# Princic-1837592/julia-raytracer

Hardware: AMD Instinct MI355X
Metric: Mrays/s + wall-clock render time, cornellbox 1280×720×256spp (higher is better)
Workload: dtype f32; 1 GPU; cornellbox path 1280x720x256spp; scene=cornellbox, sampler=path, width=1280, height=720, spp=256, bounces=8, batch=256, traversal=near, traversal_requested=auto, bvh=middle, parallelism=1 tile groups x 1 sample ranges + RCCL reduce

## Files before the change

### julia-raytracer_amd/csrc/jt_bsdf.h

```cpp
#pragma once

#include "jt_device.h"

namespace jtd {

enum { M_MATTE = 0, M_GLOSSY, M_REFLECTIVE, M_TRANSPARENT, M_REFRACTIVE, M_SUBSURFACE, M_VOLUMETRIC, M_GLTFPBR };

struct MatPoint {
    int type;
    v3 emission, color;
    float opacity, roughness, metallic, ior;
    v3 density, scattering;
    float scanisotropy, trdepth;
};

__device__ __forceinline__ v3 up_normal(v3 normal, v3 outgoing) { return dot(normal, outgoing) <= 0 ? -normal : normal; }

__device__ __forceinline__ float fresnel_dielectric(float eta, v3 normal, v3 outgoing) {
    float cosw = __builtin_fabsf(dot(normal, outgoing));
    float sin2 = 1 - cosw * cosw;
    float eta2 = eta * eta;
    float cos2t = 1 - sin2 / eta2;
    if (cos2t < 0) return 1;
    float t0 = __builtin_sqrtf(cos2t);
// ... 24 lines not shown
    float sin2 = jl_clamp(1 - cos2, 0.0f, 1.0f);
    return V3(fresnel_conductor1(eta.x, 0.0f, cosw, cos2, sin2), fresnel_conductor1(eta.y, 0.0f, cosw, cos2, sin2),
              fresnel_conductor1(eta.z, 0.0f, cosw, cos2, sin2));
}
__device__ __forceinline__ v3 reflectivity_to_eta(v3 r) {
    float a = __builtin_sqrtf(jl_clamp(r.x, 0.0f, 0.99f));
    float b = __builtin_sqrtf(jl_clamp(r.y, 0.0f, 0.99f));
    float c = __builtin_sqrtf(jl_clamp(r.z, 0.0f, 0.99f));
    return V3((1 + a) / (1 - a), (1 + b) / (1 - b), (1 + c) / (1 - c));
}
__device__ __forceinline__ m3 basis_fromz(v3 v) {
    v3 z = normalize(v);
    float sign = __builtin_copysignf(1.0f, z.z);
    float a = -1.0f / (sign + z.z);
    float b = z.x * z.y * a;
    return m3{V3(1.0f + sign * z.x * z.x * a, sign * b, -sign * z.x), V3(b, sign + z.y * z.y * a, -z.y), z};
}
__device__ __forceinline__ v3 sample_hemisphere_cos(v3 normal, v2 ruv) {
    float z = __builtin_sqrtf(ruv.y);
    float r = __builtin_sqrtf(1 - z * z);
    float phi = 2 * pif * ruv.x;
    float s, c;
    jl_sincos(phi, &s, &c);
    v3 local = V3(r * c, r * s, z);
    return normalize(mul(basis_fromz(normal), local));
}
__device__ __forceinline__ v3 sample_sphere(v2 ruv) {
    float z = 2 * ruv.y - 1;
    float r = __builtin_sqrtf(jl_clamp(1 - z * z, 0.0f, 1.0f));
    float phi = 2 * pif * ruv.x;
    float s, c;
    jl_sincos(phi, &s, &c);
    return normalize(V3(r * c, r * s, z));
}
__device__ __forceinline__ float microfacet_distribution(float roughness, v3 normal, v3 halfway) {
    float cosine = dot(normal, halfway);
    if (cosine <= 0) return 0;
    float r2 = roughness * roughness;
    float c2 = cosine * cosine;
    return r2 / (pif * (c2 * r2 + 1 - c2) * (c2 * r2 + 1 - c2));
}
__device__ __forceinline__ float microfacet_shadowing1(float roughness, v3 normal, v3 halfway, v3 direction) {
    float cosine = dot(normal, direction);
    float cosineh = dot(halfway, direction);
    if (cosine * cosineh <= 0) return 0;
    float r2 = roughness * roughness;
    float c2 = cosine * cosine;
    return 2 * __builtin_fabsf(cosine) / (__builtin_fabsf(cosine) + __builtin_sqrtf(c2 - r2 * c2 + r2));
}
__device__ __forceinline__ float microfacet_shadowing(float roughness, v3 normal, v3 halfway, v3 outgoing,
                                                      v3 incoming) {
    return microfacet_shadowing1(roughness, normal, halfway, outgoing) *
           microfacet_shadowing1(roughness, normal, halfway, incoming);
}
__device__ __forceinline__ v3 sample_microfacet(float roughness, v3 normal, v2 rn) {
    float phi = 2 * pif * rn.x;
    float theta = jl_atan(roughness * __builtin_sqrtf(rn.y / (1 - rn.y)));
    float sp, cp, st, ct;
    jl_sincos(phi, &sp, &cp);
    jl_sincos(theta, &st, &ct);
    v3 local = V3(cp * st, sp * st, ct);
    return normalize(mul(basis_fromz(normal), local));
}
__device__ __forceinline__ float sample_microfacet_pdf(float roughness, v3 normal, v3 halfway) {
    float cosine = dot(normal, halfway);
    if (cosine < 0) return 0;
// ... 243 lines not shown
}
template <int F>
__device__ __forceinline__ void eval_bsdfcos_pdf(const MatPoint& m, v3 n, v3 o, v3 i, v3& f, float& pdf) {
    f = V3(0, 0, 0);
    pdf = 0;
    if (m.roughness == 0) return;
    switch (m.type) {
        case M_MATTE:
            f = eval_matte(m.color, n, o, i);
            pdf = sample_matte_pdf(n, o, i);
            return;
        case M_GLOSSY:
            f = eval_glossy(m.color, m.ior, m.roughness, n, o, i);
            pdf = sample_glossy_pdf(m.ior, m.roughness, n, o, i);
            return;
        case M_REFLECTIVE:
            f = eval_reflective(m.color, m.roughness, n, o, i);
            pdf = sample_reflective_pdf(m.roughness, n, o, i);
            return;
        case M_TRANSPARENT:
            f = eval_transparent(m.color, m.ior, m.roughness, n, o, i);
            pdf = sample_transparent_pdf(m.ior, m.roughness, n, o, i);
            return;
        case M_REFRACTIVE:
        case M_SUBSURFACE:
            if (F & FT_VOL) {
                f = eval_refractive(m.ior, m.roughness, n, o, i);
                pdf = sample_refractive_pdf(m.ior, m.roughness, n, o, i);
            }
            return;
        default: return;
    }
}
template <int F>
__device__ __forceinline__ v3 eval_delta(const MatPoint& m, v3 n, v3 o, v3 i) {
    if (m.roughness != 0) return V3(0, 0, 0);
    switch (m.type) {
        case M_REFLECTIVE: return eval_reflective_delta(m.color, n, o, i);
        case M_TRANSPARENT: return eval_transparent_delta(m.color, m.ior, n, o, i);
        case M_REFRACTIVE: return (F & FT_VOL) ? eval_refractive_delta(m.ior, n, o, i) : V3(0, 0, 0);
        case M_VOLUMETRIC:
            return ((F & FT_VOL) && !(dot(n, i) * dot(n, o) >= 0)) ? V3(1, 1, 1) : V3(0, 0, 0);
        default: return V3(0, 0, 0);
    }
}
template <int F>
__device__ __forceinline__ v3 sample_delta(const MatPoint& m, v3 n, v3 o, float rnl) {
    if (m.roughness != 0) return V3(0, 0, 0);
    switch (m.type) {
        case M_REFLECTIVE: return reflect(o, up_normal(n, o));
        case M_TRANSPARENT: return sample_transparent_delta(m.ior, n, o, rnl);
        case M_REFRACTIVE: return (F & FT_VOL) ? sample_refractive_delta(m.ior, n, o, rnl) : V3(0, 0, 0);
        case M_VOLUMETRIC: return -o;
        default: return V3(0, 0, 0);
    }
}
template <int F>
__device__ __forceinline__ float sample_delta_pdf(const MatPoint& m, v3 n, v3 o, v3 i) {
    if (m.roughness != 0) return 0;
    switch (m.type) {
        case M_REFLECTIVE: return dot(n, i) * dot(n, o) <= 0 ? 0.0f : 1.0f;
        case M_TRANSPARENT: return sample_transparent_delta_pdf(m.ior, n, o, i);
        case M_REFRACTIVE: return (F & FT_VOL) ? sample_refractive_delta_pdf(m.ior, n, o, i) : 0.0f;
        case M_VOLUMETRIC: return dot(n, i) * dot(n, o) >= 0 ? 0.0f : 1.0f;
        default: return 0;
    }
// ... 63 lines not shown
```

### julia-raytracer_amd/csrc/jt_integrator.h

```cpp
#pragma once

#include <hip/hip_runtime.h>

#include "jt_bsdf.h"
#include "jt_device.h"
#include "jt_launch.h"
#include "jt_scene_eval.h"
#include "jt_traverse.h"

#ifndef JT_FUSED_BSDF
#define JT_FUSED_BSDF 1
#endif

namespace jtk {
using namespace jtd;

template <int F>
__device__ __forceinline__ v3 sample_lights(const DScene& S, v3 position, float rl, float rel, v2 ruv) {
    const int light_id = sample_uniform(S.nlights, rl);
    const DLight l = S.lights[light_id - 1];
    const float* cdf = S.cdf + l.cdf_offset;
    if (l.instance >= 0) {
        const int element = l.nguide ? sample_discrete_guided(cdf, l.ncdf, rel, S.guide_t + l.guide_offset,
                                                              S.guide_a + l.guide_offset, l.nguide, l.guide_scale)
// ... 256 lines not shown
        if (light_hit<F>(S, P, st, query_hit(T))) return true;
    } while (st.phase == PH_LIGHT);
    return false;
}

struct Aov {
    float* acc;
    float w_;
    int first_;
    int lk_;
    template <int F>
    __device__ __forceinline__ float w() const {
        if (!lane_lds(F)) return w_;
        if (ft_none(F)) return jl_rcp_weight((float)(((reinterpret_cast<const int*>(acc)[11 * BLOCK] - first_) >> lk_) + 1));
        return acc[12 * BLOCK];
    }
};
template <int F>
__device__ __forceinline__ void aov_update(const Aov& a, v3 ta, v3 tn) {
    const float aw = a.w<F>();
    const float omw = 1 - aw;
    float* p = a.acc;
    p[4 * BLOCK] = p[4 * BLOCK] * omw + ta.x * aw;
    p[5 * BLOCK] = p[5 * BLOCK] * omw + ta.y * aw;
    p[6 * BLOCK] = p[6 * BLOCK] * omw + ta.z * aw;
    p[7 * BLOCK] = p[7 * BLOCK] * omw + tn.x * aw;
    p[8 * BLOCK] = p[8 * BLOCK] * omw + tn.y * aw;
    p[9 * BLOCK] = p[9 * BLOCK] * omw + tn.z * aw;
}
struct NoAov {};
template <int F>
__device__ __forceinline__ void aov_update(const NoAov&, v3, v3) {}

template <int F, class AovT>
__device__ __forceinline__ bool path_hit(const DScene& S, const DParams& P, Path& st, Hit isec, const AovT& aov,
                                         unsigned& shades) {
    if (!isec.hit) {
        if (st.bounce() > 0 || !P.envhidden)
            st.set_radiance<F>(st.radiance<F>() + st.weight<F>() * eval_environment<F>(S, st.d));
        return true;
    }
    bool in_volume = false;
    if ((F & FT_VOL) && st.flag(F_VOLUME)) {
        float rl = rand1f(st.rng), rd = rand1f(st.rng);
        float distance = sample_transmittance(st.vol.density, isec.t, rl, rd);
        v3 tr = eval_transmittance(st.vol.density, distance);
        float tp = sample_transmittance_pdf(st.vol.density, distance, isec.t);
        st.set_weight<F>((st.weight<F>() * tr) / tp);
        in_volume = distance < isec.t;
        isec.t = distance;
    }
    if (!in_volume) {
        v3 outgoing = -st.d;
        Shading sh;
        eval_shading<F>(S, isec.inst, isec.elem, V2(isec.u, isec.v), outgoing, sh);
        shades++;
        if (P.nocaustics) {
            st.set_max_roughness<F>(jl_max(sh.mat.roughness, st.max_roughness<F>()));
            sh.mat.roughness = st.max_roughness<F>();
        }
        if ((F & FT_OPAC) && sh.mat.opacity < 1 && rand1f(st.rng) >= sh.mat.opacity) {
            if (st.opbounce() > 128) return true;
            st.ctl += 1u << CTL_OPB;
            st.o = sh.position + st.d * 0.01f;
            return next_bounce_retry(P, st);
        }
        if (st.bounce() == 0) {
            st.set_flag(F_HIT);
            aov_update<F>(aov, sh.mat.color, sh.normal);
        }
        st.set_radiance<F>(st.radiance<F>() + st.weight<F>() * (dot(sh.normal, outgoing) >= 0 ? sh.mat.emission : V3(0, 0, 0)));
        v3 incoming;
        const bool delta = is_delta(sh.mat);
        if (!delta) {
            if (rand1f(st.rng) < 0.5f) {
                float rnl = rand1f(st.rng);
                v2 rn = rand2f(st.rng);
                incoming = sample_bsdfcos<F>(sh.mat, sh.normal, outgoing, rnl, rn);
            } else {
                float rl = rand1f(st.rng), rel = rand1f(st.rng);
                v2 ruv = rand2f(st.rng);
                incoming = sample_lights<F>(S, sh.position, rl, rel, ruv);
            }
            if (is_zero(incoming)) return true;
#if JT_FUSED_BSDF
            v3 fb;
            float pbv;
            eval_bsdfcos_pdf<F>(sh.mat, sh.normal, outgoing, incoming, fb, pbv);
            st.set_weight<F>(st.weight<F>() * fb);
            st.set_pb<F>(pbv);
#else
            st.set_weight<F>(st.weight<F>() * eval_bsdfcos<F>(sh.mat, sh.normal, outgoing, incoming));
            st.set_pb<F>(sample_bsdfcos_pdf<F>(sh.mat, sh.normal, outgoing, incoming));
#endif
        } else {
            float rnl = rand1f(st.rng);
            incoming = sample_delta<F>(sh.mat, sh.normal, outgoing, rnl);
            v3 f = eval_delta<F>(sh.mat, sh.normal, outgoing, incoming);
            float pd = sample_delta_pdf<F>(sh.mat, sh.normal, outgoing, incoming);
            st.set_weight<F>((st.weight<F>() * f) / pd);
        }
        const int mtype = sh.mat.type;
        if ((F & FT_VOL) && (mtype == M_REFRACTIVE || mtype == M_VOLUMETRIC || mtype == M_SUBSURFACE) &&
            dot(sh.normal, outgoing) * dot(sh.normal, incoming) < 0) {
            if (!st.flag(F_VOLUME)) {
                st.set_flag(F_VOLUME);
                st.vol.density = sh.mat.density;
                st.vol.scattering = sh.mat.scattering;
                st.vol.scanisotropy = sh.mat.scanisotropy;
            } else {
                st.clear_flag(F_VOLUME);
            }
        }
        st.o = sh.position;
        st.d = incoming;
        return delta ? after_weight<F>(P, st) : begin_light_pdf<F>(S, P, st);
    }
    v3 outgoing = -st.d;
    v3 position = st.o + st.d * isec.t;
    v3 incoming;
    if (rand1f(st.rng) < 0.5f) {
        (void)rand1f(st.rng);
        v2 rn = rand2f(st.rng);
        incoming = sample_scattering(st.vol, outgoing, rn);
    } else {
        float rl = rand1f(st.rng), rel = rand1f(st.rng);
        v2 ruv = rand2f(st.rng);
        incoming = sample_lights<F>(S, position, rl, rel, ruv);
    }
    if (is_zero(incoming)) return true;
    st.set_weight<F>(st.weight<F>() * eval_scattering(st.vol, outgoing, incoming));
    st.set_pb<F>(sample_scattering_pdf(st.vol, outgoing, incoming));
    st.o = position;
    st.d = incoming;
    return begin_light_pdf<F>(S, P, st);
}

template <int F, class AovT>
__device__ __forceinline__ bool naive_hit(const DScene& S, const DParams& P, Path& st, Hit isec, const AovT& aov,
                                          unsigned& shades) {
    if (!isec.hit) {
        if (st.bounce() > 0 || !P.envhidden)
            st.set_radiance<F>(st.radiance<F>() + st.weight<F>() * eval_environment<F>(S, st.d));
        return true;
    }
    v3 outgoing = -st.d;
    Shading sh;
    eval_shading<F>(S, isec.inst, isec.elem, V2(isec.u, isec.v), outgoing, sh);
    shades++;
    if ((F & FT_OPAC) && sh.mat.opacity < 1 && rand1f(st.rng) >= sh.mat.opacity) {
        if (st.opbounce() > 128) return true;
        st.ctl += 1u << CTL_OPB;
        st.o = sh.position + st.d * 0.01f;
        return next_bounce_retry(P, st);
    }
    if (st.bounce() == 0) {
        st.set_flag(F_HIT);
        aov_update<F>(aov, sh.mat.color, sh.normal);
    }
    st.set_radiance<F>(st.radiance<F>() + st.weight<F>() * (dot(sh.normal, outgoing) >= 0 ? sh.mat.emission : V3(0, 0, 0)));
    v3 incoming, f;
    float p;
    if (sh.mat.roughness != 0) {
        float rnl = rand1f(st.rng);
        v2 rn = rand2f(st.rng);
        incoming = sample_bsdfcos<F>(sh.mat, sh.normal, outgoing, rnl, rn);
        if (is_zero(incoming)) return true;
#if JT_FUSED_BSDF
        eval_bsdfcos_pdf<F>(sh.mat, sh.normal, outgoing, incoming, f, p);
#else
        f = eval_bsdfcos<F>(sh.mat, sh.normal, outgoing, incoming);
        p = sample_bsdfcos_pdf<F>(sh.mat, sh.normal, outgoing, incoming);
#endif
    } else {
        float rnl = rand1f(st.rng);
        incoming = sample_delta<F>(sh.mat, sh.normal, outgoing, rnl);
        if (is_zero(incoming)) return true;
        f = eval_delta<F>(sh.mat, sh.normal, outgoing, incoming);
        p = sample_delta_pdf<F>(sh.mat, sh.normal, outgoing, incoming);
    }
    st.set_weight<F>((st.weight<F>() * f) / p);
    st.o = sh.position;
    st.d = incoming;
    return after_weight<F>(P, st);
}

__device__ __forceinline__ void eval_camera(const DCamera& cam, v2 image_uv, v2 lens_uv, v3& ro, v3& rd) {
    const fr3 frame = frame_from(cam.frame);
    const v2 film = V2(cam.film_x, cam.film_y);
    if (!cam.orthographic) {
        v3 q = V3(film.x * (0.5f - image_uv.x), film.y * (image_uv.y - 0.5f), cam.lens);
        v3 dc = -normalize(q);
        v3 e = V3(lens_uv.x * cam.aperture / 2, lens_uv.y * cam.aperture / 2, 0);
        v3 p = (dc * cam.focus) / __builtin_fabsf(dc.z);
        v3 d = normalize(p - e);
        ro = transform_point(frame, e);
        rd = transform_direction(frame, d);
    } else {
        float scale = 1 / cam.lens;
        v3 q = V3(film.x * (0.5f - image_uv.x) * scale, film.y * (image_uv.y - 0.5f) * scale, cam.lens);
        v3 e = V3(-q.x, -q.y, 0) + V3(lens_uv.x * cam.aperture / 2, lens_uv.y * cam.aperture / 2, 0);
        v3 p = V3(-q.x, -q.y, -cam.focus);
// ... 34 lines not shown
```

### julia-raytracer_amd/csrc/jt_kernels.h

```cpp
#pragma once

#include <hip/hip_runtime.h>

#include <algorithm>

#include "jt_integrator.h"
#include "jt_launch.h"

namespace jtk {
using namespace jtd;

#ifndef JT_STAMPS
#define JT_STAMPS 0
#endif
#ifndef JT_NODE_REPEAT_NONE
#define JT_NODE_REPEAT_NONE 4
#endif
#ifndef JT_NODE_REPEAT
#define JT_NODE_REPEAT 3
#endif
#ifndef JT_FIRST_POP_NONE
#define JT_FIRST_POP_NONE 1
#endif
#ifndef JT_FIRST_POP
// ... 114 lines not shown
template <int F>
__device__ __forceinline__ unsigned item_of(int ut, int l, int i, int j) {
    return item_coords<F>() ? item_encode(i, j) : (unsigned)(ut * 64 + l);
}
template <int F>
__device__ __forceinline__ int item_pixel_index(unsigned item, const DParams& P, int tiles_x) {
    return item_coords<F>() ? item_j(item) * P.width + item_i(item) : item_pixel(item, P, tiles_x);
}
template <int F>
__device__ __forceinline__ int item_slot(unsigned item, const DParams& P) {
    if constexpr (item_coords<F>()) return item_slot(item, (P.width + 7) >> 3, P.tile_offset, P.tile_stride_rcp);
    else {
        const float inv = __uint_as_float(__builtin_amdgcn_readfirstlane(__float_as_uint(1.0f / (float)P.tile_stride)));
        return launch_tile((int)(item >> 6), P.tile_offset, inv) * 64 + (int)(item & 63u);
    }
}
__device__ __forceinline__ float stream_weight(const DParams& P, int s) {
    return jl_rcp_weight((float)(((s - P.first) >> P.lk) + 1));
}

#if JT_STAMPS
#define JT_STAMP(x) x
#else
#define JT_STAMP(x)
#endif

template <int SAMPLER, int RING, bool OVF, int COUNT, int F, bool NCACHE, bool WIDE, bool ADAPT = false>
__device__ __forceinline__ void trace_body_items(const DScene& S0, const DParams& P0, int s_begin, int s_end,
                                                 const DAccum& A, int* stack) {
    const DScene& S = S0;
    const DParams& P = P0;
    static_assert(lane_lds(F), "the per-lane item body keeps the lane's sample index in LDS");
    constexpr int PB = push_bit(node_baked<OVF, NCACHE, WIDE, F>());
    const int lane = threadIdx.x & 63;
    const int oslot = (int)blockIdx.x * BLOCK + (int)threadIdx.x;
    if constexpr ((F & (FT_TEX | FT_ENV)) != 0) {
        for (int k = threadIdx.x; k < 512; k += BLOCK) tex_lut[k] = k < 256 ? S.srgb_lut[k] : S.byte_lut[k - 256];
        __syncthreads();
    }
    Counters cnt{0, 0, 0, 0};
    constexpr bool WC = !ft_none(F);
    unsigned w_paths = 0, w_rays = 0, w_lq = 0;
    __shared__ unsigned wave_cnt[WC ? 1 : (BLOCK / 64) * 4];
    unsigned* const wcnt = wave_cnt + (WC ? 0 : (threadIdx.x >> 6) * 4);
    if (!WC && lane < 3) wcnt[lane] = 0u;
    auto lds_count = [&](int k, bool c) {
        if (c) __hip_atomic_fetch_add(wcnt + k, 1u, __ATOMIC_RELAXED, __HIP_MEMORY_SCOPE_WORKGROUP);
    };
    __shared__ float acc_lds[acc_slots(F) * BLOCK];
    float* acc = acc_lds + threadIdx.x;
    int* const acc_i = reinterpret_cast<int*>(acc);
#if JT_STAMPS
    unsigned long long t_trav = 0, t_shade = 0, n_trav = 0, n_shade = 0, lanes_p = 0, lanes_n = 0, steps_p = 0, steps_n = 0;
    unsigned long long t_hit = 0, t_fin = 0, t_qb = 0, n_phit = 0, n_fin = 0, idle = 0, n_mph = 0, n_mty = 0, n_mid = 0;
    unsigned long long lanes_sh = 0, lanes_hit = 0, t_start = 0, n_start = 0, lanes_start = 0;
#endif
    const int tiles_x = (P.width + 7) / 8, tiles = launch_tiles(P);
    const int kstr = 1 << P.lk;
    const int nq = s_end - s_begin < kstr ? s_end - s_begin : kstr;
    unsigned xcc;
    asm volatile("s_getreg_b32 %0, hwreg(HW_REG_XCC_ID)" : "=s"(xcc));
    int band_k = 0;
    int ut = 0, uq = 0, bnext = 64;
    bool drained = false;
    unsigned item = ITEM_NONE;
    bool next_sample = false;
// ... 180 lines not shown
                n_mph++;
                lanes_hit += lane_count(__builtin_amdgcn_ballot_w64(mt >= 0));
                for (int ty = 0; ty <= (int)M_GLTFPBR; ty++) n_mty += __builtin_amdgcn_ballot_w64(mt == ty) ? 1u : 0u;
                bool counted = mt < 0;
                for (;;) {
                    const unsigned long long m = __builtin_amdgcn_ballot_w64(!counted);
                    if (!m) break;
                    const int v = __shfl(mid, __ffsll((long long)m) - 1);
                    counted = counted || mid == v;
                    n_mid++;
                }
            }
        }
        unsigned long long ts3 = ts2, ts4 = ts2;
#endif
        constexpr bool LINL = (F & (FT_LINL | FT_NOIL)) != 0;
        {
            const bool tie = query_done<WIDE>(T) && (T.nh & (TIE_SEEN | REF_RERUN)) == TIE_SEEN &&
                             !(LSTEP && st.phase == PH_FINISH);
            if (S.order_flip && __builtin_amdgcn_ballot_w64(tie))
                if (tie) rerun_tie<WIDE>(S, T, st.o, st.d, SAMPLER == 1 && !LINL && st.phase == PH_LIGHT ? S.lights[st.li].instance : -1, stack, PB);
        }
        bool c_path = false, c_lq = false, c_ray = false;
        unsigned n_inl = 0;
        if (query_done<WIDE>(T)) {
            const DParams& P = karg_params<karg_params_on<SAMPLER, F>()>(P0);
            const DScene SL = shade_scene_lds<NCACHE, RING, OVF, F>(S0);
            const DScene& S = NCACHE ? shade_scene<karg_scene<NCACHE, F>()>(S0) : SL;
            bool alive = true;
            const bool light = SAMPLER == 1 && !LINL && st.phase == PH_LIGHT;
            bool done;
            if (LSTEP && st.phase == PH_FINISH) done = true;
            else if (light) done = light_hit<F>(S, P, st, query_hit(T));
            else if (SAMPLER == 2) done = naive_hit<F>(S, P, st, query_hit(T), aov, cnt.shades);
            else done = path_hit<F>(S, P, st, query_hit(T), aov, cnt.shades);
            bool chained = false;
            if (SAMPLER == 1 && !done && st.phase == PH_LIGHT && chains_inline(F, S)) {
                unsigned nlq = 0;
                chained = true;
                done = light_chain<WIDE, RING, OVF, COUNT, NCACHE, F>(S, P, st, T, stack, oslot, cnt, [&] {
                    if (WC) nlq++;
                    else lds_count(2, true);
                });
                if (WC) n_inl += nlq;
            }
#if JT_STAMPS
            ts3 = __builtin_amdgcn_s_memtime();
            n_phit++;
#endif
            if (done) {
                if (WC) c_path = true;
                else lds_count(0, true);
                v3 radiance = st.radiance<F>();
                if (!all_finite(radiance)) radiance = V3(0, 0, 0);
                const float mr = max3(radiance);
                if (mr > P.clamp) radiance = radiance * (P.clamp / mr);
                const float w = aov.w<F>();
                const float omw = 1 - w;
                const bool hit = st.flag(F_HIT);
                const bool env = !hit && !P.envhidden && S.nenvs != 0;
                const v4 target = (hit || env) ? V4(radiance.x, radiance.y, radiance.z, 1) : V4(0, 0, 0, 0);
                if (!hit) aov_update<F>(aov, env ? V3(1, 1, 1) : V3(0, 0, 0), -st.d);
                acc[0] = acc[0] * omw + target.x * w;
                acc[BLOCK] = acc[BLOCK] * omw + target.y * w;
                acc[2 * BLOCK] = acc[2 * BLOCK] * omw + target.z * w;
                acc[3 * BLOCK] = acc[3 * BLOCK] * omw + target.w * w;
                if (hit || env) acc_i[10 * BLOCK] += 1;
                alive = false;
// ... 106 lines not shown
    L.enrm_id = reinterpret_cast<const float4*>(blob + S.o_enrm_id);
    L.materials = reinterpret_cast<const DMaterial*>(blob + S.o_materials);
    L.lights = reinterpret_cast<const DLight*>(blob + S.o_lights);
    L.light_hit = reinterpret_cast<const int4*>(blob + S.o_light_hit);
    L.light_elems = reinterpret_cast<const float4*>(blob + S.o_light_elems);
    L.cdf = reinterpret_cast<const float*>(blob + S.o_cdf);
    return L;
}

__device__ __forceinline__ void bake_nodes(const DScene& S, uint4* blob) {
    uint4* const nodes = blob + S.o_nodes;
    const int nnodes = (S.o_wnodes - S.o_nodes) >> 1;
    const int iroot0 = JT_INST_ROOTS ? instance_root_base(S.o_nodes, S.o_inst_trav) : 0;
    for (int k = threadIdx.x; k < nnodes; k += BLOCK) {
        uint4& b = nodes[2 * k + 1];
        const BakedNode bn = bake_node(b.w, (int)b.z, k < S.tlas_nnodes ? T_TLAS : T_BLAS, iroot0);
        b.z = bn.e0;
        b.w = bn.meta;
    }
    if (JT_INST_ROOTS) {
        const int ninst = (S.o_inst_blas - S.o_inst_trav) >> 2;
        for (int i = threadIdx.x; i < ninst; i += BLOCK) {
            const uint4* const root = S.blob + S.o_nodes + 2 * (int)S.blob[S.o_inst_blas + i].x;
            uint4 b = root[1];
            const BakedNode bn = bake_node(b.w, (int)b.z, T_BLAS);
            b.z = bn.e0;
            b.w = bn.meta;
            nodes[2 * (iroot0 + i)] = root[0];
            nodes[2 * (iroot0 + i) + 1] = b;
        }
    }
}

template <int SAMPLER, int RING, bool OVF, int COUNT, int F, bool WIDE, bool ADAPT>
__global__ __launch_bounds__(BLOCK) JT_WAVES_PER_EU void trace_kernel(DScene S, DParams P, int s_begin, int s_end, DAccum A) {
    __shared__ int lds_stack[RING * BLOCK];
    trace_body_items<SAMPLER, RING, OVF, COUNT, F, true, WIDE, ADAPT>(S, P, s_begin, s_end, A, lds_stack + threadIdx.x);
}

template <int SAMPLER, int RING, bool OVF, int COUNT, int F, bool WIDE, bool ADAPT>
__global__ __launch_bounds__(BLOCK) JT_WAVES_PER_EU_F(F) void trace_kernel_lds(DScene S, DParams P, int s_begin, int s_end, DAccum A) {
    extern __shared__ uint4 dyn_lds[];
    uint4* blob = dyn_lds + lds_stack_bytes(OVF, RING, S.stack_need) / 16;
    for (int k = threadIdx.x; k < S.blob_n16; k += BLOCK) blob[k] = S.blob[k];
    __syncthreads();
    if constexpr (node_baked<OVF, false, WIDE, F>()) {
        bake_nodes(S, blob);
        __syncthreads();
    }
    const DScene L = blob_scene(S, blob);
    trace_body_items<SAMPLER, RING, OVF, COUNT, F, false, WIDE, ADAPT>(L, P, s_begin, s_end, A, reinterpret_cast<int*>(dyn_lds) + threadIdx.x);
}

template <int SAMPLER, int RING, bool OVF, int COUNT, int F, bool LDSK, bool WIDE, bool ADAPT>
hipError_t launch_t(const DScene& S, const DParams& P, int s0, int s1, const DAccum& A, hipStream_t st, int cus) {
    const long long units = (long long)launch_tiles(P) * std::min(s1 - s0, 1 << P.lk);
    const int want = (int)std::min<long long>((units + BLOCK / 64 - 1) / (BLOCK / 64), 1 << 30);
    if (want == 0) return hipSuccess;
    int per_cu = 0;
    hipError_t e;
    if constexpr (LDSK) {
        if (S.blob_n16 > 0) {
        const size_t lds = lds_stack_bytes(OVF, RING, S.stack_need) + (size_t)S.blob_n16 * 16;
        constexpr auto kl = &trace_kernel_lds<SAMPLER, RING, OVF, COUNT, F, WIDE, ADAPT>;
        const void* k = (const void*)kl;
        if ((e = hipFuncSetAttribute(k, hipFuncAttributeMaxDynamicSharedMemorySize, (int)lds)) != hipSuccess) return e;
        if (hipOccupancyMaxActiveBlocksPerMultiprocessor(&per_cu, k, BLOCK, lds) != hipSuccess || per_cu < 1) per_cu = 1;
        const int nwg = std::min(want, std::min(per_cu, 8) * cus);
        hipLaunchKernelGGL(kl, dim3(nwg), dim3(BLOCK), lds, st, S, P, s0, s1, A);
        return hipGetLastError();
        }
    }
    constexpr auto kh = &trace_kernel<SAMPLER, RING, OVF, COUNT, F, WIDE, ADAPT>;
    const void* k = (const void*)kh;
    if (hipOccupancyMaxActiveBlocksPerMultiprocessor(&per_cu, k, BLOCK, 0) != hipSuccess || per_cu < 1) per_cu = 1;
    const int nwg = std::min(want, std::min(per_cu, 8) * cus);
    hipLaunchKernelGGL(kh, dim3(nwg), dim3(BLOCK), 0, st, S, P, s0, s1, A);
    return hipGetLastError();
}

// ... 8 lines not shown
```

### julia-raytracer_amd/csrc/jt_layout.cpp

```cpp
#include "jt_layout.h"

#include <algorithm>
#include <cmath>
#include <cstdlib>
#include <cstring>
#include <functional>
#include <string>
#include <vector>

using namespace jtd;

namespace jt {
namespace {

inline float4 f4(float x, float y, float z, float w) { return make_float4(x, y, z, w); }
template <class I>
inline float as_f(I v) {
    static_assert(sizeof(I) == 4, "32-bit integers only");
    float f;
    std::memcpy(&f, &v, 4);
    return f;
}

void build_alias_table(const float* cdf, int n, std::vector<float2>& out) {
// ... 455 lines not shown
                const int* v = &sh.quads[4 * el];
                const jt::f3 a = vertex(sh, v[0]), b = vertex(sh, v[1]), cc = vertex(sh, v[2]), dd = vertex(sh, v[3]);
                const bool degenerate = cc.x == dd.x && cc.y == dd.y && cc.z == dd.z;
                prims.push_back(f4(a.x, a.y, a.z, as_f(el)));
                prims.push_back(f4(b.x, b.y, b.z, 0));
                prims.push_back(f4(cc.x, cc.y, cc.z, 0));
                prims.push_back(f4(dd.x, dd.y, dd.z, degenerate ? 1.0f : 0.0f));
            }
        }
    }
}

void flatten_instances(const jt_scene* scene, const jt_scene_bvh* bvh, HostScene& hs) {
    hs.inst_trav.resize(scene->ninstances);
    hs.inst_blas.resize(scene->ninstances);
    hs.inst_shade.resize(scene->ninstances);
    for (int k0 = 0; k0 < scene->ninstances; k0++) {
        const int k = hs.inst_new[k0];
        const jt_instance& in = scene->instances[k0];
        jt::frame3 f = jt::load_frame(in.frame);
        jt::frame3 inv = jt::inverse_frame(f, true);
        float iv[12], fv[12];
        jt::store_frame(inv, iv);
        jt::store_frame(f, fv);
        const DShape& d = hs.shapes[in.shape];
        hs.inst_trav[k] = DInstTrav{f4(iv[0], iv[1], iv[2], iv[3]), f4(iv[4], iv[5], iv[6], iv[7]), f4(iv[8], iv[9], iv[10], iv[11]),
                                    in.shape, d.blas_root, d.kind, d.prim_base};
        const float idm[12] = {1, 0, 0, 0, 1, 0, 0, 0, 1, 0, 0, 0};
        bool ident = true;
        for (int q = 0; q < 12; q++) ident = ident && iv[q] == idm[q];
        const jt_bvh_tree& bt = bvh->blas[in.shape];
        const bool leaf_root = bt.nnodes > 0 && !bt.nodes[0].internal;
        hs.inst_blas[k] = make_int4(hs.wide ? hs.wroot[in.shape] : d.blas_root, ident ? 1 : 0, d.kind, in.shape | (leaf_root ? 1 << 30 : 0));
        if (!ident) hs.feat |= FT_XFORM;
        hs.inst_shade[k] = DInstShade{f4(fv[0], fv[1], fv[2], fv[3]), f4(fv[4], fv[5], fv[6], fv[7]), f4(fv[8], fv[9], fv[10], fv[11]),
                                      in.material, in.shape, scene->materials[in.material].type,
                                      rot_identity(fv) ? 1 : 0};
    }
}

int flatten_materials(const jt_scene* scene, HostScene& hs) {
    hs.materials.resize(scene->nmaterials);
    for (int k = 0; k < scene->nmaterials; k++) {
        const jt_material& m = scene->materials[k];
        DMaterial& d = hs.materials[k];
        std::memset(&d, 0, sizeof(d));
        d.type = m.type;
        d.emission_tex = m.emission_tex;
        d.color_tex = m.color_tex;
        d.roughness_tex = m.roughness_tex;
        d.scattering_tex = m.scattering_tex;
        d.normal_tex = m.normal_tex;
        for (int q = 0; q < 3; q++) {
            d.emission[q] = m.emission[q];
            d.color[q] = m.color[q];
            d.scattering[q] = m.scattering[q];
        }
        d.roughness = m.roughness;
        d.metallic = m.metallic;
        d.ior = m.ior;
        d.scanisotropy = m.scanisotropy;
        d.trdepth = m.trdepth;
        d.opacity = m.opacity;
    }
    hs.textures.resize(scene->ntextures);
    for (int k = 0; k < scene->ntextures; k++) {
        const jt_texture& t = scene->textures[k];
// ... 189 lines not shown
```

### julia-raytracer_amd/csrc/jt_scene_eval.h

```cpp
#pragma once

#include <hip/hip_runtime.h>

#include "jt_bsdf.h"
#include "jt_device.h"

namespace jtk {
using namespace jtd;

template <int F>
__device__ __forceinline__ int4 row16(const void* p) {
    int4 v = *reinterpret_cast<const int4*>(p);
    if (!ft_none(F)) __asm__("" : "+v"(v.x), "+v"(v.y), "+v"(v.z), "+v"(v.w));
    return v;
}
template <int F>
__device__ __forceinline__ int4 inst_ids(const DScene& S, int inst) {
    return row16<F>(reinterpret_cast<const char*>(S.inst_shade + inst) + 48);
}
__device__ __forceinline__ fr3 inst_frame(const DScene& S, int inst) {
    const DInstShade& r = S.inst_shade[inst];
    return frame_from(r.f0, r.f1, r.f2);
}

// ... 114 lines not shown
                                          const DMaterial& m, v2 uv) {
    v3 normal = eval_normal(S, sh, e, f, uv);
    v2 texcoord = eval_texcoord(S, sh, e, uv);
    v4 t4 = eval_texture(S, m.normal_tex, texcoord, false);
    v3 nm = V3(t4.x * 2 - 1, t4.y * 2 - 1, t4.z * 2 - 1);
    v3 tu = V3(0, 0, 0), tv = V3(0, 0, 0);
    if (sh.tc_base >= 0) {
        const int b = sh.tc_base - sh.pos_base;
        float2 a1 = S.tc[e.x + b], a2 = S.tc[e.y + b];
        if (sh.kind == KIND_TRI) {
            float2 a3 = S.tc[e.z + b];
            triangle_tangents_fromuv(xyz(S.pos[e.x]), xyz(S.pos[e.y]), xyz(S.pos[e.z]), V2(a1.x, a1.y),
                                     V2(a2.x, a2.y), V2(a3.x, a3.y), tu, tv);
        } else {
            float2 a4 = S.tc[e.w + b];
            triangle_tangents_fromuv(xyz(S.pos[e.x]), xyz(S.pos[e.y]), xyz(S.pos[e.w]), V2(a1.x, a1.y),
                                     V2(a2.x, a2.y), V2(a4.x, a4.y), tu, tv);
        }
        tu = transform_direction(f, tu);
        tv = transform_direction(f, tv);
    }
    v3 f1 = normalize(tu - normal * dot(tu, normal));
    v3 f2 = normalize(cross(normal, tu));
    bool flip_v = dot(f2, tv) < 0;
    nm = V3(nm.x, nm.y * (flip_v ? 1.0f : -1.0f), nm.z);
    fr3 fr{f1, f2, normal, V3(0, 0, 0)};
    return transform_normal(fr, nm);
}

struct Shading {
    v3 position, normal;
    MatPoint mat;
};

template <int F>
__device__ __forceinline__ void eval_shading(const DScene& S, int inst, int elem, v2 uv, v3 outgoing, Shading& out) {
    const DInstShade is = S.inst_shade[inst];
    const DShape sh = S.shapes[is.shape];
    const int4 e = S.elems[sh.idx_base + elem];
    const fr3 f = frame_from(is.f0, is.f1, is.f2);
    const DMaterial& m = S.materials[is.material];
    v3 p1 = xyz(S.pos[e.x]), p2 = xyz(S.pos[e.y]), p3 = xyz(S.pos[e.z]);
    const bool tri = !(F & FT_QUAD) || sh.kind == KIND_TRI;
    v3 p4 = !tri ? xyz(S.pos[e.w]) : p3;
    out.position = tri ? transform_point(f, interp_tri(p1, p2, p3, uv))
                       : transform_point(f, interp_quad(p1, p2, p3, p4, uv));
    const int mtype = (F & FT_MAT) ? m.type : (int)M_MATTE;
    v3 normal;
    if ((F & FT_TEX) && m.normal_tex >= 0) {
        normal = eval_normalmap(S, sh, e, f, m, uv);
    } else if (!(F & FT_ATTR) || sh.nrm_base < 0) {
        normal = element_normal(S, is.rot_identity, f, sh.idx_base + elem);
    } else {
        normal = eval_normal(S, sh, e, f, uv);
    }
    if (mtype != M_REFRACTIVE) normal = dot(normal, outgoing) >= 0 ? normal : -normal;
    out.normal = normal;
    MatPoint& p = out.mat;
    const v4 one = V4(1, 1, 1, 1);
    v2 texcoord = (F & FT_ATTR) ? eval_texcoord(S, sh, e, uv) : uv;
    v4 emission_tex = (F & FT_TEX) ? eval_texture(S, m.emission_tex, texcoord, true) : one;
    v4 color_shp = (F & FT_ATTR) ? eval_color(S, sh, e, uv) : one;
    v4 color_tex = (F & FT_TEX) ? eval_texture(S, m.color_tex, texcoord, true) : one;
    v4 roughness_tex = (F & FT_TEX) ? eval_texture(S, m.roughness_tex, texcoord, false) : one;
    v4 scattering_tex = (F & FT_TEX) ? eval_texture(S, m.scattering_tex, texcoord, true) : one;
    p.type = mtype;
    p.emission = V3(m.emission[0], m.emission[1], m.emission[2]) * xyz(emission_tex);
    p.color = (V3(m.color[0], m.color[1], m.color[2]) * xyz(color_tex)) * xyz(color_shp);
    p.opacity = m.opacity * color_tex.w * color_shp.w;
    p.metallic = m.metallic * roughness_tex.z;
    float roughness = m.roughness * roughness_tex.y;
    roughness = roughness * roughness;
    p.ior = m.ior;
    p.scattering = V3(m.scattering[0], m.scattering[1], m.scattering[2]) * xyz(scattering_tex);
    p.scanisotropy = m.scanisotropy;
    p.trdepth = m.trdepth;
    if ((F & FT_VOL) && (mtype == M_REFRACTIVE || mtype == M_VOLUMETRIC || mtype == M_SUBSURFACE)) {
        p.density = V3(-jl_log(jl_clamp(p.color.x, 0.0001f, 1.0f)) / p.trdepth,
                       -jl_log(jl_clamp(p.color.y, 0.0001f, 1.0f)) / p.trdepth,
                       -jl_log(jl_clamp(p.color.z, 0.0001f, 1.0f)) / p.trdepth);
    } else {
        p.density = V3(0, 0, 0);
    }
    if (mtype == M_MATTE || mtype == M_GLTFPBR || mtype == M_GLOSSY) roughness = jl_clamp(roughness, min_roughness, 1.0f);
    else if (mtype == M_VOLUMETRIC) roughness = 0.0f;
    else if (roughness < min_roughness) roughness = 0.0f;
    p.roughness = roughness;
}

template <int F>
__device__ __forceinline__ v3 eval_environment(const DScene& S, v3 direction) {
    v3 emission = V3(0, 0, 0);
    if (!(F & FT_ENV)) return emission;
    for (int k = 0; k < S.nenvs; k++) {
        const DEnv& env = S.envs[k];
        v3 wl = transform_direction(frame_from(env.inv), direction);
        v2 tc = V2(jl_atan2(wl.z, wl.x) / (2.0f * pif), jl_acos(jl_clamp(wl.y, -1.0f, 1.0f)) / pif);
        if (tc.x < 0.0f) tc.x = tc.x + 1.0f;
        v4 t = eval_texture(S, env.tex, tc, false);
        emission = emission + V3(env.emission[0], env.emission[1], env.emission[2]) * xyz(t);
    }
    return emission;
}

}
```

### julia-raytracer_amd/csrc/jt_traverse.h

```cpp
#pragma once

#include <hip/hip_runtime.h>

#include "jt_device.h"
#include "jt_launch.h"
#include "jt_push.h"

#ifndef JT_CHILD_PRETEST
#define JT_CHILD_PRETEST 1
#endif

namespace jtk {
using namespace jtd;


struct Hit {
    int inst, elem;
    float u, v, t;
    bool hit;
};
struct Counters {
    unsigned nodes, instances, prims, shades;
};

// ... 5 lines not shown
    int low;
    int inst_space;
    int negmask;
    int cur_inst, cur_kind;
    int prim, nprim;
    int h_inst, h_elem;
    float h_u, h_v;
    int nh;
    unsigned nxt;
};

#ifndef JT_TIE_RERUN
#define JT_TIE_RERUN 1
#endif
constexpr int TIE_SEEN = 1 << 8, REF_RERUN = 1 << 9, NH_COUNT = 63;
__device__ __forceinline__ int query_flip(const DScene& S, const Trav& T, int pb = 0) {
    return ((T.nh & REF_RERUN) ? 0 : S.order_flip) | pb;
}
__device__ __forceinline__ void hit_count(Trav& T, float t) {
    T.nh = (T.nh + ((T.nh & NH_COUNT) < NH_COUNT ? 1 : 0)) | (JT_TIE_RERUN && t == T.tmax ? TIE_SEEN : 0);
}

#ifndef JT_NODE_BAKE
#define JT_NODE_BAKE 1
#endif
#ifndef JT_NODE_READ16
#define JT_NODE_READ16 0
#endif
template <bool OVF, bool NCACHE, bool WIDE, int F>
__host__ __device__ constexpr bool node_baked() {
    return JT_NODE_BAKE && !OVF && !NCACHE && !WIDE && ft_none(F);
}
__host__ __device__ constexpr int push_bit(bool baked) { return baked ? BAKE_MASK_BIT : 0; }
#ifndef JT_INST_ROOTS
#define JT_INST_ROOTS 1
#endif
__device__ __forceinline__ int inst_root_base(const DScene& S, int pb) {
    return JT_INST_ROOTS && pb ? instance_root_base(S.o_nodes, S.o_inst_trav) : 0;
}

__device__ __forceinline__ int neg_mask(v3 d, int flip) {
    return ((d.x < 0 ? 1 : 0) | (d.y < 0 ? 2 : 0) | (d.z < 0 ? 4 : 0)) ^ flip;
}

__device__ __forceinline__ void world_ray(const DScene& S, Trav& T, int pb = 0) {
    T.lo = T.wo;
    T.ld = T.wd;
    T.ldinv = T.wdinv;
    T.negmask = neg_mask(T.wd, query_flip(S, T, pb));
    T.inst_space = 0;
}

__device__ __forceinline__ Hit query_hit(const Trav& T) {
    return Hit{T.h_inst, T.h_elem, T.h_u, T.h_v, T.tmax, T.h_inst >= 0};
}

__device__ __forceinline__ bool query_busy(const Trav& T) { return T.sp > 0 || T.nprim > 0; }
template <bool WIDE>
__device__ __forceinline__ bool wants_node(const Trav& T) {
    return T.nprim == 0 && (T.sp > 0 || (WIDE && T.nxt != W_EMPTY));
}
template <bool WIDE>
__device__ __forceinline__ bool query_done(const Trav& T) {
    return (T.sp | T.nprim) == 0 && (!WIDE || T.nxt == W_EMPTY);
}

// ... 382 lines not shown
```

Baseline: 13930 Mrays/s.

## Bake per-element shading basis and color/pi into LDS blob for matte-only kernels

When node baking is active for feature-free scenes, each block precomputes per-element orthonormal basis terms and per-material color/pi into spare slots of the LDS scene blob. The path and naive integrators then sample the cosine hemisphere and evaluate the matte BSDF from these baked values, skipping the basis_fromz math and generic material dispatch. The baked path treats every material as matte and reuses the scattering field to hold color/pi, which only holds for FT_NONE scenes. Instances whose rotation is not identity are now flagged FT_XFORM so they stay off this path. The cost is extra per-block setup work and a larger dependence on scene layout assumptions.

```diff
diff --git a/julia-raytracer_amd/csrc/jt_bsdf.h b/julia-raytracer_amd/csrc/jt_bsdf.h
--- a/julia-raytracer_amd/csrc/jt_bsdf.h
+++ b/julia-raytracer_amd/csrc/jt_bsdf.h
@@ -80,6 +80,33 @@
     float s, c;
     jl_sincos(phi, &s, &c);
     return normalize(V3(r * c, r * s, z));
+}
+
+struct BakedBasis {
+    v3 n;
+    float xx, yx, yy;
+    v3 z;
+};
+__device__ __forceinline__ m3 basis_baked(const BakedBasis& k, bool flip) {
+    const v3 z = flip ? -k.z : k.z;
+    const float b = flip ? -k.yx : k.yx;
+    const float sign = __builtin_copysignf(1.0f, z.z);
+    return m3{V3(k.xx, sign * b, -sign * z.x), V3(b, flip ? 0.0f - k.yy : k.yy, -z.y), z};
+}
+template <class Load>
+__device__ __forceinline__ v3 sample_matte_baked(Load load, float roughness, v3 outgoing, v2 rn) {
+    if (roughness == 0) return V3(0, 0, 0);
+    float z = __builtin_sqrtf(rn.y);
+    float r = __builtin_sqrtf(1 - z * z);
+    float phi = 2 * pif * rn.x;
+    float s, c;
+    jl_sincos(phi, &s, &c);
+    const v3 local = V3(r * c, r * s, z);
+    __asm__ volatile("" ::: "memory");
+    const BakedBasis k = load();
+    const bool flip = !(dot(k.n, outgoing) >= 0);
+    const v3 normal = flip ? -k.n : k.n;
+    return normalize(mul(basis_baked(k, flip != (dot(normal, outgoing) <= 0)), local));
 }
 __device__ __forceinline__ float microfacet_distribution(float roughness, v3 normal, v3 halfway) {
     float cosine = dot(normal, halfway);
@@ -389,6 +416,13 @@
         default: return;
     }
 }
+__device__ __forceinline__ void eval_matte_pdf_baked(v3 color_pi, float roughness, v3 n, v3 o, v3 i, v3& f, float& pdf) {
+    f = V3(0, 0, 0);
+    pdf = 0;
+    if (roughness == 0) return;
+    if (!(dot(n, i) * dot(n, o) <= 0)) f = color_pi * __builtin_fabsf(dot(n, i));
+    pdf = sample_matte_pdf(n, o, i);
+}
 template <int F>
 __device__ __forceinline__ v3 eval_delta(const MatPoint& m, v3 n, v3 o, v3 i) {
     if (m.roughness != 0) return V3(0, 0, 0);
diff --git a/julia-raytracer_amd/csrc/jt_integrator.h b/julia-raytracer_amd/csrc/jt_integrator.h
--- a/julia-raytracer_amd/csrc/jt_integrator.h
+++ b/julia-raytracer_amd/csrc/jt_integrator.h
@@ -312,7 +312,7 @@
 template <int F>
 __device__ __forceinline__ void aov_update(const NoAov&, v3, v3) {}
 
-template <int F, class AovT>
+template <int F, bool SB = false, class AovT>
 __device__ __forceinline__ bool path_hit(const DScene& S, const DParams& P, Path& st, Hit isec, const AovT& aov,
                                          unsigned& shades) {
     if (!isec.hit) {
@@ -333,7 +333,8 @@
     if (!in_volume) {
         v3 outgoing = -st.d;
         Shading sh;
-        eval_shading<F>(S, isec.inst, isec.elem, V2(isec.u, isec.v), outgoing, sh);
+        BakedShade bk;
+        eval_shading<F, SB>(S, isec.inst, isec.elem, V2(isec.u, isec.v), outgoing, sh, &bk);
         shades++;
         if (P.nocaustics) {
             st.set_max_roughness<F>(jl_max(sh.mat.roughness, st.max_roughness<F>()));
@@ -356,7 +357,8 @@
             if (rand1f(st.rng) < 0.5f) {
                 float rnl = rand1f(st.rng);
                 v2 rn = rand2f(st.rng);
-                incoming = sample_bsdfcos<F>(sh.mat, sh.normal, outgoing, rnl, rn);
+                if constexpr (SB) incoming = sample_matte_baked([&] { return baked_basis(S, bk.elem); }, sh.mat.roughness, outgoing, rn);
+                else incoming = sample_bsdfcos<F>(sh.mat, sh.normal, outgoing, rnl, rn);
             } else {
                 float rl = rand1f(st.rng), rel = rand1f(st.rng);
                 v2 ruv = rand2f(st.rng);
@@ -366,7 +368,8 @@
 #if JT_FUSED_BSDF
             v3 fb;
             float pbv;
-            eval_bsdfcos_pdf<F>(sh.mat, sh.normal, outgoing, incoming, fb, pbv);
+            if constexpr (SB) eval_matte_pdf_baked(baked_color_pi(S, bk.material), sh.mat.roughness, sh.normal, outgoing, incoming, fb, pbv);
+            else eval_bsdfcos_pdf<F>(sh.mat, sh.normal, outgoing, incoming, fb, pbv);
             st.set_weight<F>(st.weight<F>() * fb);
             st.set_pb<F>(pbv);
 #else
@@ -416,7 +419,7 @@
     return begin_light_pdf<F>(S, P, st);
 }
 
-template <int F, class AovT>
+template <int F, bool SB = false, class AovT>
 __device__ __forceinline__ bool naive_hit(const DScene& S, const DParams& P, Path& st, Hit isec, const AovT& aov,
                                           unsigned& shades) {
     if (!isec.hit) {
@@ -426,7 +429,8 @@
     }
     v3 outgoing = -st.d;
     Shading sh;
-    eval_shading<F>(S, isec.inst, isec.elem, V2(isec.u, isec.v), outgoing, sh);
+    BakedShade bk;
+    eval_shading<F, SB>(S, isec.inst, isec.elem, V2(isec.u, isec.v), outgoing, sh, &bk);
     shades++;
     if ((F & FT_OPAC) && sh.mat.opacity < 1 && rand1f(st.rng) >= sh.mat.opacity) {
         if (st.opbounce() > 128) return true;
@@ -444,10 +448,12 @@
     if (sh.mat.roughness != 0) {
         float rnl = rand1f(st.rng);
         v2 rn = rand2f(st.rng);
-        incoming = sample_bsdfcos<F>(sh.mat, sh.normal, outgoing, rnl, rn);
+        if constexpr (SB) incoming = sample_matte_baked([&] { return baked_basis(S, bk.elem); }, sh.mat.roughness, outgoing, rn);
+        else incoming = sample_bsdfcos<F>(sh.mat, sh.normal, outgoing, rnl, rn);
         if (is_zero(incoming)) return true;
 #if JT_FUSED_BSDF
-        eval_bsdfcos_pdf<F>(sh.mat, sh.normal, outgoing, incoming, f, p);
+        if constexpr (SB) eval_matte_pdf_baked(baked_color_pi(S, bk.material), sh.mat.roughness, sh.normal, outgoing, incoming, f, p);
+        else eval_bsdfcos_pdf<F>(sh.mat, sh.normal, outgoing, incoming, f, p);
 #else
         f = eval_bsdfcos<F>(sh.mat, sh.normal, outgoing, incoming);
         p = sample_bsdfcos_pdf<F>(sh.mat, sh.normal, outgoing, incoming);
diff --git a/julia-raytracer_amd/csrc/jt_kernels.h b/julia-raytracer_amd/csrc/jt_kernels.h
--- a/julia-raytracer_amd/csrc/jt_kernels.h
+++ b/julia-raytracer_amd/csrc/jt_kernels.h
@@ -170,6 +170,7 @@
     const DParams& P = P0;
     static_assert(lane_lds(F), "the per-lane item body keeps the lane's sample index in LDS");
     constexpr int PB = push_bit(node_baked<OVF, NCACHE, WIDE, F>());
+    constexpr bool SB = shade_baked<OVF, NCACHE, WIDE, F>();
     const int lane = threadIdx.x & 63;
     const int oslot = (int)blockIdx.x * BLOCK + (int)threadIdx.x;
     if constexpr ((F & (FT_TEX | FT_ENV)) != 0) {
@@ -416,8 +417,8 @@
             bool done;
             if (LSTEP && st.phase == PH_FINISH) done = true;
             else if (light) done = light_hit<F>(S, P, st, query_hit(T));
-            else if (SAMPLER == 2) done = naive_hit<F>(S, P, st, query_hit(T), aov, cnt.shades);
-            else done = path_hit<F>(S, P, st, query_hit(T), aov, cnt.shades);
+            else if (SAMPLER == 2) done = naive_hit<F, SB>(S, P, st, query_hit(T), aov, cnt.shades);
+            else done = path_hit<F, SB>(S, P, st, query_hit(T), aov, cnt.shades);
             bool chained = false;
             if (SAMPLER == 1 && !done && st.phase == PH_LIGHT && chains_inline(F, S)) {
                 unsigned nlq = 0;
@@ -590,6 +591,26 @@
     }
 }
 
+__device__ __forceinline__ void bake_shading(const DScene& S, uint4* blob) {
+    static_assert(sizeof(DMaterial) == 6 * 16, "six 16-B units per material");
+    const int nelem = S.o_enrm_id - S.o_enrm;
+    for (int g = threadIdx.x; g < nelem; g += BLOCK) {
+        float4& ni = reinterpret_cast<float4*>(blob + S.o_enrm_id)[g];
+        const m3 b = basis_fromz(xyz(ni));
+        reinterpret_cast<float4*>(blob + S.o_enrm)[g] = make_float4(b.c3.x, b.c3.y, b.c3.z, b.c1.x);
+        ni.w = b.c2.x;
+        blob[S.o_elems + g].w = __float_as_uint(b.c2.y);
+    }
+    const int nmat = (S.o_lights - S.o_materials) / 6;
+    for (int k = threadIdx.x; k < nmat; k += BLOCK) {
+        DMaterial& m = reinterpret_cast<DMaterial*>(blob + S.o_materials)[k];
+        const v3 c = V3(m.color[0], m.color[1], m.color[2]) / pif;
+        m.scattering[0] = c.x;
+        m.scattering[1] = c.y;
+        m.scattering[2] = c.z;
+    }
+}
+
 template <int SAMPLER, int RING, bool OVF, int COUNT, int F, bool WIDE, bool ADAPT>
 __global__ __launch_bounds__(BLOCK) JT_WAVES_PER_EU void trace_kernel(DScene S, DParams P, int s_begin, int s_end, DAccum A) {
     __shared__ int lds_stack[RING * BLOCK];
@@ -604,6 +625,7 @@
     __syncthreads();
     if constexpr (node_baked<OVF, false, WIDE, F>()) {
         bake_nodes(S, blob);
+        if constexpr (shade_baked<OVF, false, WIDE, F>()) bake_shading(S, blob);
         __syncthreads();
     }
     const DScene L = blob_scene(S, blob);
diff --git a/julia-raytracer_amd/csrc/jt_layout.cpp b/julia-raytracer_amd/csrc/jt_layout.cpp
--- a/julia-raytracer_amd/csrc/jt_layout.cpp
+++ b/julia-raytracer_amd/csrc/jt_layout.cpp
@@ -511,7 +511,7 @@
         const jt_bvh_tree& bt = bvh->blas[in.shape];
         const bool leaf_root = bt.nnodes > 0 && !bt.nodes[0].internal;
         hs.inst_blas[k] = make_int4(hs.wide ? hs.wroot[in.shape] : d.blas_root, ident ? 1 : 0, d.kind, in.shape | (leaf_root ? 1 << 30 : 0));
-        if (!ident) hs.feat |= FT_XFORM;
+        if (!ident || !rot_identity(fv)) hs.feat |= FT_XFORM;
         hs.inst_shade[k] = DInstShade{f4(fv[0], fv[1], fv[2], fv[3]), f4(fv[4], fv[5], fv[6], fv[7]), f4(fv[8], fv[9], fv[10], fv[11]),
                                       in.material, in.shape, scene->materials[in.material].type,
                                       rot_identity(fv) ? 1 : 0};
diff --git a/julia-raytracer_amd/csrc/jt_scene_eval.h b/julia-raytracer_amd/csrc/jt_scene_eval.h
--- a/julia-raytracer_amd/csrc/jt_scene_eval.h
+++ b/julia-raytracer_amd/csrc/jt_scene_eval.h
@@ -170,9 +170,22 @@
     v3 position, normal;
     MatPoint mat;
 };
-
-template <int F>
-__device__ __forceinline__ void eval_shading(const DScene& S, int inst, int elem, v2 uv, v3 outgoing, Shading& out) {
+struct BakedShade {
+    int elem, material;
+};
+__device__ __forceinline__ BakedBasis baked_basis(const DScene& S, int g) {
+    const float4 bz = S.enrm[g], ni = S.enrm_id[g];
+    return BakedBasis{xyz(ni), bz.w, ni.w, __int_as_float(S.elems[g].w), xyz(bz)};
+}
+__device__ __forceinline__ v3 baked_color_pi(const DScene& S, int material) {
+    const DMaterial& m = S.materials[material];
+    return V3(m.scattering[0], m.scattering[1], m.scattering[2]);
+}
+
+template <int F, bool SB = false>
+__device__ __forceinline__ void eval_shading(const DScene& S, int inst, int elem, v2 uv, v3 outgoing, Shading& out,
+                                             BakedShade* bk = nullptr) {
+    static_assert(!SB || ft_none(F), "baked shading: the FT_NONE kernels only");
     const DInstShade is = S.inst_shade[inst];
     const DShape sh = S.shapes[is.shape];
     const int4 e = S.elems[sh.idx_base + elem];
@@ -187,6 +200,10 @@
     v3 normal;
     if ((F & FT_TEX) && m.normal_tex >= 0) {
         normal = eval_normalmap(S, sh, e, f, m, uv);
+    } else if constexpr (SB) {
+        normal = xyz(S.enrm_id[sh.idx_base + elem]);
+        bk->elem = sh.idx_base + elem;
+        bk->material = is.material;
     } else if (!(F & FT_ATTR) || sh.nrm_base < 0) {
         normal = element_normal(S, is.rot_identity, f, sh.idx_base + elem);
     } else {
@@ -210,7 +227,7 @@
     float roughness = m.roughness * roughness_tex.y;
     roughness = roughness * roughness;
     p.ior = m.ior;
-    p.scattering = V3(m.scattering[0], m.scattering[1], m.scattering[2]) * xyz(scattering_tex);
+    p.scattering = SB ? V3(0, 0, 0) : V3(m.scattering[0], m.scattering[1], m.scattering[2]) * xyz(scattering_tex);
     p.scanisotropy = m.scanisotropy;
     p.trdepth = m.trdepth;
     if ((F & FT_VOL) && (mtype == M_REFRACTIVE || mtype == M_VOLUMETRIC || mtype == M_SUBSURFACE)) {
diff --git a/julia-raytracer_amd/csrc/jt_traverse.h b/julia-raytracer_amd/csrc/jt_traverse.h
--- a/julia-raytracer_amd/csrc/jt_traverse.h
+++ b/julia-raytracer_amd/csrc/jt_traverse.h
@@ -61,6 +61,13 @@
     return JT_NODE_BAKE && !OVF && !NCACHE && !WIDE && ft_none(F);
 }
 __host__ __device__ constexpr int push_bit(bool baked) { return baked ? BAKE_MASK_BIT : 0; }
+#ifndef JT_SHADE_BAKE
+#define JT_SHADE_BAKE 1
+#endif
+template <bool OVF, bool NCACHE, bool WIDE, int F>
+__host__ __device__ constexpr bool shade_baked() {
+    return JT_SHADE_BAKE && node_baked<OVF, NCACHE, WIDE, F>();
+}
 #ifndef JT_INST_ROOTS
 #define JT_INST_ROOTS 1
 #endif
```

Result: faster. 14150 Mrays/s, median of 6 (+1.6%).
